# sergiventosa/ts-PWS

Measured on AMD Instinct MI355X. Metric: stacked samples/s (Morlet ts-PWS, 10k×131072) + % HBM roofline, 1/2/4/8 GPU, higher is better.
Workload: dtype f64; 1 GPU; 10000 traces/GPU x 131072 samples, Morlet w0=pi*sqrt(2/ln2) V=4 J=14, two-stage K=10 + unbiased phase coherence (BASELINE configs[2]); HBM-resident float32 traces; traces_total=10000, traces_per_gpu=10000, parallelism=one GPU: no collective, world_size=1

## Files before the change

### ts-pws_amd/csrc/inv_poly.h

```cpp
#pragma once

#define INV_R 8
#ifndef INV_UNIFORM
#define INV_UNIFORM 1
#endif

#ifndef FL_ABLATE
#define FL_ABLATE 0
#endif
#if FL_ABLATE
__device__ unsigned inv_class_mask = 0x7fu;
#endif

#define INV_QB 32
#define INV_WROWS (64 * INV_R + INV_QB + 16)
#define INV_WPAD(e) ((e) + ((e) >> 3))
#define INV_SLAB (INV_WROWS + INV_WROWS / 8 + 2)

struct OctDesc {
	unsigned s0, nv;
	unsigned D, Ns;
	unsigned DL, logDL, MC;
	unsigned ngw;
	unsigned wave_off;
	unsigned slot;
	unsigned gen, pad1;
};

#define INV_QSTEP(TP, YW)                                                                                     \
	if constexpr (QUAD) {                                                                                     \
		_Pragma("unroll") for (int c = 0; c < NREC; c++)                                                      \
			_Pragma("unroll") for (int r = 0; r < R; r++)                                                     \
				accq[c][r] = fma((TP).x, (YW).y, fma(-(TP).y, (YW).x, accq[c][r]));                             \
	}
template <int NREC, bool GEN, bool LDSW = false, bool QUAD = false>
__global__ void __launch_bounds__(256) k_inv_poly(const double2 *__restrict__ Y, size_t ncoef, unsigned N, const ScaleDesc *__restrict__ sc,
                                                  const OctDesc *__restrict__ oc, unsigned noct, const double2 *__restrict__ wd,
                                                  double *__restrict__ obuf, size_t slot_stride, unsigned total_waves, size_t y_coef,
                                                  size_t y_obuf, unsigned wave_base, size_t q_off = 0)
{
	Y += (size_t)blockIdx.y * y_coef; obuf += (size_t)blockIdx.y * y_obuf;
	constexpr int R = INV_R;
	const unsigned lane = threadIdx.x & 63;
	const unsigned wid = wave_base + blockIdx.x * 4 + __builtin_amdgcn_readfirstlane(threadIdx.x >> 6);
	if (wid >= total_waves) return;
	unsigned lo = 0, hi = noct;
	while (hi - lo > 1) {
		const unsigned mid = (lo + hi) >> 1;
		if (oc[mid].wave_off <= wid) lo = mid; else hi = mid;
	}
	const OctDesc o = oc[lo];
#if FL_ABLATE
	if (!((inv_class_mask >> o.logDL) & 1u)) return;
#endif
	const unsigned wl = wid - o.wave_off;
	const unsigned chunk = wl / o.ngw, gb = wl - chunk * o.ngw;
	const unsigned n0 = chunk * 64 + (lane & (o.DL - 1));
	const unsigned g = gb * (64u / o.DL) + (lane >> o.logDL);
	const bool live = n0 < o.D && g * R < o.Ns;
	const unsigned n0c = n0 < o.D ? n0 : 0;
	const unsigned D = o.D, Ns = o.Ns;

	double acc[NREC][R];
#pragma unroll
	for (int c = 0; c < NREC; c++)
#pragma unroll
		for (int r = 0; r < R; r++) acc[c][r] = 0;
	double accq[QUAD ? NREC : 1][R];
#pragma unroll
// ... 86 lines not shown
#pragma unroll
				for (int j = 0; j < R - 1; j++) {
					const bool in = idx >= 0 && idx < (long long)Ns;
#pragma unroll
					for (int c = 0; c < NREC; c++) yw[c][j] = in ? ys[(size_t)c * ncoef + (size_t)(in ? idx : 0)] : make_double2(0.0, 0.0);
					idx++;
				}
				unsigned l = mu;
				for (unsigned q = 0; q < d.Q + 1; q += R) {
#pragma unroll
					for (int u = 0; u < R; u++) {
						const bool in = idx >= 0 && idx < (long long)Ns;
#pragma unroll
						for (int c = 0; c < NREC; c++)
							yw[c][(u + R - 1) % R] = in ? ys[(size_t)c * ncoef + (size_t)(in ? idx : 0)] : make_double2(0.0, 0.0);
						idx++;
						double2 tp = ws[l < d.L ? l : d.L - 1];
						if (l < d.L) {
							tp.x *= gD; tp.y *= gD;
#pragma unroll
							for (int c = 0; c < NREC; c++)
#pragma unroll
								for (int r = 0; r < R; r++)
									acc[c][r] = fma(tp.x, yw[c][(u + r) % R].x, fma(tp.y, yw[c][(u + r) % R].y, acc[c][r]));
							INV_QSTEP(tp, yw[c][(u + r) % R])
						}
						l += D;
					}
				}
			}
		}
	} else if (INV_UNIFORM && o.DL == 64) {
	const unsigned gu = gb;
	for (unsigned v = 0; v < o.nv; v++) {
		const ScaleDesc d = sc[o.s0 + v];
		const double2 *ws = wd + d.tap_off;
		const double2 *ys = Y + d.coef_off;
		const long long t = (long long)n0c - d.cd;
		const long long a = t >= 0 ? t / D : -((-t + D - 1) / D);
		const unsigned rho = (unsigned)(t - a * (long long)D);
		const unsigned mu = rho ? D - rho : 0;
		const int idx = (int)a + (rho ? 1 : 0);
		const int A = __builtin_amdgcn_readfirstlane(idx);
		const unsigned shift = n0 < D ? (unsigned)(idx - A) : 0u;
		long long am = ((long long)A + (long long)gu * R) % (long long)Ns;
		if (am < 0) am += Ns;
		unsigned row = (unsigned)am;
		const double gD = d.gain * (double)D;
		double2 yw[NREC][R];
#pragma unroll
		for (int j = 0; j < R - 1; j++) {
#pragma unroll
			for (int c = 0; c < NREC; c++) yw[c][j] = ys[(size_t)c * ncoef + row];
			if (++row == Ns) row = 0;
		}
		unsigned l = mu - shift * D;
		for (unsigned q = 0; q < d.Q + 1; q += R) {
#pragma unroll
			for (int u = 0; u < R; u++) {
#pragma unroll
				for (int c = 0; c < NREC; c++) yw[c][(u + R - 1) % R] = ys[(size_t)c * ncoef + row];
				if (++row == Ns) row = 0;
				double2 tp = ws[l < d.L ? l : d.L - 1];
				if (l < d.L) {
					tp.x *= gD; tp.y *= gD;
#pragma unroll
					for (int c = 0; c < NREC; c++)
#pragma unroll
						for (int r = 0; r < R; r++)
							acc[c][r] = fma(tp.x, yw[c][(u + r) % R].x, fma(tp.y, yw[c][(u + r) % R].y, acc[c][r]));
					INV_QSTEP(tp, yw[c][(u + r) % R])
				}
				l += D;
			}
		}
	}
	} else {
	for (unsigned v = 0; v < o.nv; v++) {
		const ScaleDesc d = sc[o.s0 + v];
		const double2 *ws = wd + d.tap_off;
		const double2 *ys = Y + d.coef_off;
		const long long t = (long long)n0c - d.cd;
		long long a = t >= 0 ? t / D : -((-t + D - 1) / D);
		const unsigned rho = (unsigned)(t - a * (long long)D);
		const unsigned mu = rho ? D - rho : 0;
		a += (long long)g * R + (rho ? 1 : 0);
		long long am = a % (long long)Ns;
		if (am < 0) am += Ns;
		unsigned row = (unsigned)am;
		const double gD = d.gain * (double)D;
		double2 yw[NREC][R];
#pragma unroll
		for (int j = 0; j < R - 1; j++) {
#pragma unroll
			for (int c = 0; c < NREC; c++) yw[c][j] = ys[(size_t)c * ncoef + row];
			if (++row == Ns) row = 0;
		}
		unsigned l = mu, q = 0;
		for (; q + R <= d.Q; q += R) {
#pragma unroll
			for (int u = 0; u < R; u++) {
#pragma unroll
				for (int c = 0; c < NREC; c++) yw[c][(u + R - 1) % R] = ys[(size_t)c * ncoef + row];
				if (++row == Ns) row = 0;
				double2 tp = ws[l < d.L ? l : d.L - 1];
				if (l < d.L) {
					tp.x *= gD; tp.y *= gD;
#pragma unroll
// ... 149 lines not shown
```

### ts-pws_amd/csrc/forward.hip

```cpp
#include "tspws_internal.h"
#include <type_traits>

#ifndef FL_PASSES
#define FL_PASSES 2
#endif
#ifndef FL_WAVES
#define FL_WAVES 4
#endif
#ifndef FL_PASSES_FINE
#define FL_PASSES_FINE 1
#endif

template <typename TIn, bool BLOCK_PER_OUT>
__global__ void __launch_bounds__(256) k_fwd_generic(const TIn *__restrict__ x, size_t ld, unsigned N, const ScaleDesc *__restrict__ sc,
                                                     unsigned S, const double2 *__restrict__ w, double2 *__restrict__ Y, size_t ncoef,
                                                     unsigned long long first_coef, unsigned long long n_items)
{
	__shared__ double red[8];
	const unsigned lane = threadIdx.x & 63, wv = threadIdx.x >> 6;
	unsigned long long item = BLOCK_PER_OUT ? blockIdx.x : (unsigned long long)blockIdx.x * 4 + wv;
	if (item >= n_items) return;
	const unsigned long long ci = first_coef + item;
	const unsigned s = find_scale(sc, S, ci, false);
	const ScaleDesc d = sc[s];
// ... 22 lines not shown
			re = red[0] + red[2] + red[4] + red[6];
			im = red[1] + red[3] + red[5] + red[7];
			*out = make_double2(re, -im);
		}
	} else if (lane == 0) *out = make_double2(re, -im);
}

template <typename TIn>
static int forward_generic(tspws_hip_plan *p, const TIn *d_x, size_t ntr, size_t ld, double *d_Y, hipStream_t st)
{
	if (!p || !d_x || !d_Y) return fail(TSPWS_E_ARG, "forward: NULL");
	if (!ntr) return 0;
	HIP_TRY(hipSetDevice(p->device));
	unsigned s_long = p->S;
	for (unsigned s = 0; s < p->S; s++) if (p->sc[s].L > 2048) { s_long = s; break; }
	const unsigned long long n_short = s_long < p->S ? p->sc[s_long].coef_off : p->ncoef;
	const unsigned long long n_long = p->ncoef - n_short;
	for (size_t t0 = 0; t0 < ntr; t0 += 65535) {
		const unsigned ny = (unsigned)std::min<size_t>(ntr - t0, 65535);
		const TIn *xx = d_x + t0 * ld;
		double2 *yy = (double2 *)d_Y + t0 * p->ncoef;
		if (n_long)
			hipLaunchKernelGGL((k_fwd_generic<TIn, true>), dim3((unsigned)n_long, ny), dim3(256), 0, st, xx, ld, p->N, p->d_sc, p->S,
			                   p->d_w, yy, p->ncoef, n_short, n_long);
		if (n_short)
			hipLaunchKernelGGL((k_fwd_generic<TIn, false>), dim3((unsigned)((n_short + 3) / 4), ny), dim3(256), 0, st, xx, ld, p->N,
			                   p->d_sc, p->S, p->d_w, yy, p->ncoef, 0ull, n_short);
	}
	HIP_TRY(hipGetLastError());
	return 0;
}

#include "fwd_poly.h"
#include "fwd_lds.h"
#include "fwd_tl.h"
#include "fwd_gemm.h"
#include "spectral.h"

int tspws_engine_pin()
{
	static int eng = -2;
	if (eng == -2) {
		const char *e = getenv("TSPWS_ENGINE");
		eng = (!e || !*e || !strcmp(e, "auto")) ? 0 : !strcmp(e, "fir") ? 1 : !strcmp(e, "spectral") ? 2 : -1;
	}
	return eng;
}

static long tl_min_env()
{
	const char *e = sweep_env("TSPWS_TL_MIN");
	return e ? std::max(1, atoi(e)) : -1;
}

#ifndef FWD_LDS_MIN_NG
#define FWD_LDS_MIN_NG 8
#endif
#ifndef TL_MINNS0
#define TL_MINNS0 33
#endif
#ifndef FWD_STEPS_DEF
#define FWD_STEPS_DEF 32
#endif
#ifndef FWD_STEPS_TL
#define FWD_STEPS_TL 96
#endif
static int build_tl_forward(tspws_hip_plan *p, unsigned FWD_STEPS, unsigned MINNS, unsigned TLSTEPS, TlTable &T, unsigned spec_first = ~0u, unsigned spec_end = ~0u,
                            unsigned nblk_hint = 0);

int tspws_build_forward(tspws_hip_plan *p)
{
	const unsigned S = p->S;
	unsigned FWD_STEPS = FWD_STEPS_DEF;
	if (const char *e = sweep_env("TSPWS_FWD_STEPS")) FWD_STEPS = (unsigned)std::max(8, atoi(e));
	const unsigned R = 8, FL_SLOTS_HOST = FL_WAVES * FL_PASSES;
	unsigned woff = 0, boff = 0;
	unsigned long long poff = 0;
	for (unsigned s = 0; s < S; s++) {
		ScaleDesc &d = p->sc[s];
		d.Q = (d.L + d.D - 1) / d.D;
		unsigned dl = 1, lg = 0;
		while (dl < d.D && dl < 64) { dl <<= 1; lg++; }
		d.DL = dl; d.logDL = lg;
		d.MC = d.D > 64 ? (d.D + 63) / 64 : 1;
		const unsigned NG = (d.Ns + R - 1) / R, GW = 64 / d.DL;
		const bool pow2 = (d.D & (d.D - 1)) == 0;
		d.use_lds = (NG >= FWD_LDS_MIN_NG && (d.D >= 64 || pow2)) ? 1u : 0u;
		d.ngw = (NG + GW - 1) / GW;
		d.r16 = (!d.use_lds && d.DL == 64 && d.Ns >= 16) ? 1u : 0u;
		if (d.r16) d.ngw = (d.Ns + 15) / 16;
		unsigned cps;
		if (d.use_lds) cps = 1;
		else cps = std::max(1u, (FWD_STEPS + d.Q / 2) / std::max(1u, d.Q));
		d.cps = std::min(cps, d.MC);
		d.nsplit = (d.MC + d.cps - 1) / d.cps;
		d.wave_off = woff; d.lds_off = boff; d.part_off = poff;
		const unsigned slots = (d.D <= 4) ? FL_WAVES * FL_PASSES_FINE : FL_SLOTS_HOST;
		d.lds_bps = (NG + slots * GW - 1) / (slots * GW);
		if (d.use_lds) boff += d.lds_bps * d.nsplit; else woff += d.ngw * d.nsplit;
		poff += (unsigned long long)d.nsplit * d.Ns;
		d.fuse_ok = (d.use_lds && d.nsplit == 1) ? 1u : 0u;
		p->n_fusable += d.fuse_ok;
	}
	p->fwd_waves = woff; p->lds_blocks = boff; p->npart = poff;
	p->lds_qt = 24;
	for (unsigned s = 0; s < S; s++) if (p->sc[s].use_lds && p->sc[s].Q > 24 && p->sc[s].Q <= 32) p->lds_qt = 32;
	if (const char *e = sweep_env("TSPWS_FWD_QT")) { const int v = atoi(e); if (v == 24 || v == 32) p->lds_qt = (unsigned)v; }
	if (int rc = build_tl_forward(p, FWD_STEPS_TL, TL_MINNS0, 96, p->tl[0])) return rc;
	unsigned minns1 = 129, tlsteps1 = 48;
	if (const char *e = sweep_env("TSPWS_TLSTEPS")) tlsteps1 = (unsigned)std::max(8, atoi(e));
	if (const char *e = sweep_env("TSPWS_TL_MINNS1")) minns1 = (unsigned)std::max(9, atoi(e));
	return build_tl_forward(p, FWD_STEPS_TL, minns1, tlsteps1, p->tl[1]);
}

static int build_tl_forward(tspws_hip_plan *p, unsigned FWD_STEPS, unsigned MINNS, unsigned TLSTEPS, TlTable &T, unsigned spec_first, unsigned spec_end,
                            unsigned nblk_hint)
{
	T.minns = MINNS;
	T.sc = p->sc;
	std::vector<TLItem> items;
	std::vector<char> is_tl(p->S, 0);
	unsigned wg = 0;
	const unsigned S_fir = std::min(p->S, spec_first);
	for (unsigned s = 0; s < S_fir;) {
		unsigned e = s + 1;
		while (e < S_fir && p->sc[e].D == p->sc[s].D && p->sc[e].Ns == p->sc[s].Ns) e++;
		const unsigned D = p->sc[s].D, Ns = p->sc[s].Ns, nv = e - s;
		bool ok = Ns >= MINNS;
		std::vector<unsigned> a(nv), b(nv), qr(nv);
		for (unsigned v = 0; v < nv && ok; v++) {
			const ScaleDesc &d = p->sc[s + v];
			a[v] = (unsigned)d.c / D; b[v] = (unsigned)d.c % D;
			const long long num = (long long)d.L - 1 - (long long)b[v];
			const long long fl = num >= 0 ? num / (long long)D : -1;
			qr[v] = ((unsigned)(fl + 2) + 3) & ~3u;
			if (qr[v] > TL_QMAX) ok = false;
		}
// ... 72 lines not shown
	HIP_TRY(hipMalloc(&T.d_sc, p->S * sizeof(ScaleDesc)));
	HIP_TRY(hipMemcpy(T.d_sc, T.sc.data(), p->S * sizeof(ScaleDesc), hipMemcpyHostToDevice));
	if (T.gcoltiles) {
		std::vector<GemmCol> gc((size_t)T.gcoltiles * 16);
		memset(gc.data(), 0, gc.size() * sizeof(GemmCol));
		size_t i = 0;
		for (unsigned s = spec_end; s < p->S; s++) {
			const ScaleDesc &d = T.sc[s];
			for (unsigned k = 0; k < d.Ns; k++, i++) {
				GemmCol &g = gc[i];
				long long o = ((long long)d.c - (long long)k * (long long)d.D) % (long long)p->N;
				if (o < 0) o += p->N;
				g.L = d.L; g.o = (unsigned)o; g.Ns = d.Ns; g.tap_off = d.tap_off; g.dst = d.part_off + k;
			}
		}
		HIP_TRY(hipMalloc(&T.d_gcols, gc.size() * sizeof(GemmCol)));
		HIP_TRY(hipMemcpy(T.d_gcols, gc.data(), gc.size() * sizeof(GemmCol), hipMemcpyHostToDevice));
	}
	if (!T.n) return 0;
	HIP_TRY(hipMalloc(&T.d_items, items.size() * sizeof(TLItem)));
	HIP_TRY(hipMemcpy(T.d_items, items.data(), items.size() * sizeof(TLItem), hipMemcpyHostToDevice));
	HIP_TRY(hipFuncSetAttribute((const void *)k_fwd_tl<float>, hipFuncAttributeMaxDynamicSharedMemorySize, 160 * 1024));
	HIP_TRY(hipFuncSetAttribute((const void *)k_fwd_tl<double>, hipFuncAttributeMaxDynamicSharedMemorySize, 160 * 1024));
	return 0;
}

int tspws_build_tl_spectral(tspws_hip_plan *p, unsigned s_first, unsigned s_end, unsigned nblk_hint, TlTable &T)
{
	unsigned steps = 12;
	if (const char *e = sweep_env("TSPWS_SPEC_TLSTEPS")) steps = (unsigned)std::max(1, atoi(e));
	return build_tl_forward(p, FWD_STEPS_TL, TL_MINNS0, steps, T, s_first, s_end, nblk_hint);
}

struct LaunchRange { unsigned lds0, lds1, wav0, wav1, acc0, acc1; };
static LaunchRange launch_range(const tspws_hip_plan *p, ScaleRange rg)
{
	LaunchRange r;
	r.lds0 = rg.on() ? p->sc[rg.s0].lds_off : 0u;
	r.lds1 = rg.on() && rg.s1 < p->S ? p->sc[rg.s1].lds_off : p->lds_blocks;
	r.wav0 = rg.on() ? p->sc[rg.s0].wave_off : 0u;
	r.wav1 = rg.on() && rg.s1 < p->S ? p->sc[rg.s1].wave_off : p->fwd_waves;
	r.acc0 = rg.on() ? p->sc[rg.s0].acc2_off : 0u;
	r.acc1 = rg.on() && rg.s1 < p->S ? p->sc[rg.s1].acc2_off : p->acc2_blocks;
	return r;
}

template <typename TIn>
static void launch_poly2(const tspws_hip_plan *p, const TIn *d_x, size_t ld, size_t ntr, const ScaleDesc *d_sc, double2 *d_part, size_t npart, unsigned wav1,
                         unsigned wav0, hipStream_t st)
{
	for (size_t t0 = 0; t0 < ntr; t0 += 2 * 32768) {
		const unsigned nt = (unsigned)std::min<size_t>(ntr - t0, 2 * 32768);
		hipLaunchKernelGGL((k_fwd_poly<TIn, 2>), dim3((wav1 - wav0 + 3) / 4, (nt + 1) / 2), dim3(256), 0, st, d_x + t0 * ld, ld, nt, p->N, d_sc, p->S, p->d_w,
		                   d_part + t0 * npart, npart, wav1, wav0);
	}
}

template <typename TIn>
int tspws_forward_parts(tspws_hip_plan *p, const TIn *d_x, size_t ntr, size_t ld, double2 *d_part, hipStream_t st, FuseOut *fz, ScaleRange rg)
{
	if (fz) { fz->applied = false; fz->spec_first = p->S; }
	bool spec_join = false;
	hipStream_t fir = st;
	if constexpr (std::is_same<TIn, double>::value) {
		if (fz && fz->allow_spec && !rg.on() && fz->fin.OUT && fz->fin.nprev == 0 && ntr <= 512 && fz->tps) {
			static int min_rows = -1;
			static unsigned nsmax_env = 0;
			if (min_rows < 0) {
				const char *e = sweep_env("TSPWS_FEW_SPEC_MIN"); min_rows = e ? std::max(1, atoi(e)) : 64;
				if (const char *m = sweep_env("TSPWS_FEW_NSMAX")) nsmax_env = (unsigned)std::max(2, atoi(m));
			}
			if (ntr >= (size_t)min_rows && tspws_engine_pin() != 1 && !tspws_generic_forward()) {
				const unsigned sf = tspws_spectral_first_scale(p, nsmax_env ? nsmax_env : std::max(512u, (p->N + 15u) / 16u));
				if (sf < p->S && tspws_spectral_end_scale(p) == p->S) {
					SpecDecomp *dc = nullptr;
					int rc;
					if ((rc = tspws_spectral_decomp(p, sf, (unsigned)((ntr + 63) / 64), &dc, true))) return rc;
					static const bool serial = sweep_env("TSPWS_SPEC_PARALLEL") && !strcmp(sweep_env("TSPWS_SPEC_PARALLEL"), "0");
					hipEvent_t behind_tr = nullptr;
					if (!serial && sf > 0) {
						if ((rc = tspws_plan_stream(p, p->xs)) || (rc = tspws_plan_event(p->ev_xs2))) return rc;
						behind_tr = fz->ev_mid ? fz->ev_mid : p->ev_xs2;
					}
					if ((rc = tspws_spectral_rows_f64(p, dc, (const double *)d_x, ld, (unsigned)ntr, fz->tps, *fz, st, behind_tr))) return rc;
					fz->spec_first = sf;
					if (behind_tr) {
						if ((rc = tspws_fork(p, st, p->xs, p->ev_xs2, behind_tr))) return rc;
						fz->mid_recorded = behind_tr == fz->ev_mid;
						fir = p->xs;
					} else if (fz->ev_mid) { HIP_TRY(hipEventRecord(fz->ev_mid, st)); fz->mid_recorded = true; }
					if (sf == 0) { fz->applied = true; return 0; }
					rg.s0 = 0; rg.s1 = sf;
					spec_join = fir != st;
				}
			}
		}
	}
	const LaunchRange lr = launch_range(p, rg);
	const bool has_lds = lr.lds1 > lr.lds0, has_poly = lr.wav1 > lr.wav0;
	hipStream_t sp = fir;
#if FL_TIMING || FL_ABLATE
	static const bool serial = sweep_env("TSPWS_FWD_SERIAL") != nullptr;
#else
	constexpr bool serial = false;
#endif
	if (has_lds && has_poly && !serial) {
		if (int rc = tspws_fork(p, fir, p->side, p->ev_fork, fir == st ? p->le.ready : nullptr)) return rc;
		sp = p->side;
	}
	p->le.ready = nullptr;
	if (has_poly) {
		if (ntr == 1)
			hipLaunchKernelGGL((k_fwd_poly<TIn, 1>), dim3((lr.wav1 - lr.wav0 + 3) / 4, 1), dim3(256), 0, sp, d_x, ld, 1u, p->N, p->d_sc, p->S, p->d_w, d_part,
			                   p->npart, lr.wav1, lr.wav0);
		else launch_poly2<TIn>(p, d_x, ld, ntr, p->d_sc, d_part, p->npart, lr.wav1, lr.wav0, sp);
	}
	if (has_lds) {
		const bool fuse = fz && fz->accST && p->n_fusable;
		unsigned tps = (unsigned)std::min<size_t>(ntr, 32);
		while (tps > 1 && (size_t)p->lds_blocks * ((ntr + tps - 1) / tps) < 2048) tps = (tps + 1) / 2;
		if (fuse) tps = fz->tps;
		const size_t per_launch = (size_t)tps * 65535;
		for (size_t t0 = 0; t0 < ntr; t0 += per_launch) {
			const unsigned nt = (unsigned)std::min<size_t>(ntr - t0, per_launch);
			const dim3 grid(lr.lds1 - lr.lds0, (nt + tps - 1) / tps);
			double2 *aS = fuse ? fz->accST + (t0 / tps) * fz->stride : nullptr, *aP = fuse ? fz->accPS + (t0 / tps) * fz->stride : nullptr;
			const size_t astr = fuse ? fz->stride : 0;
			FuseFinal ff;
			if (fuse && fz->fin.OUT && t0 == 0 && ntr <= per_launch) ff = fz->fin;
#define FL_LAUNCH(F, QT) hipLaunchKernelGGL((k_fwd_lds<TIn, F, QT>), grid, dim3(FL_NT), FL_LDS_BYTES_(QT), fir, d_x + t0 * ld, ld, nt, tps, p->N, p->d_sc, p->S, \
			                            p->d_w, d_part + t0 * p->npart, p->npart, aS, aP, astr, lr.lds0, ff)
			if (p->lds_qt == 32) { if (fuse) FL_LAUNCH(true, 32); else FL_LAUNCH(false, 32); }
			else { if (fuse) FL_LAUNCH(true, 24); else FL_LAUNCH(false, 24); }
#undef FL_LAUNCH
		}
		if (fuse) fz->applied = true;
	}
	if (sp != fir) if (int rc = tspws_join(sp, fir, p->ev_join)) return rc;
	if (spec_join) {
		if (fz && fz->defer_fir_join) fz->fir_stream = p->xs;
		else if (int rc = tspws_join(p->xs, st, p->ev_xs1)) return rc;
	}
	HIP_TRY(hipGetLastError());
	return 0;
// ... 369 lines not shown
```

### ts-pws_amd/csrc/plan.hip

```cpp
#include "tspws_internal.h"

static thread_local std::string g_err;

extern "C" const char *tspws_hip_last_error(void) { return g_err.c_str(); }

int tspws_fail(int code, const char *what, hipError_t e)
{
	g_err = what;
	if (e != hipSuccess) { g_err += ": "; g_err += hipGetErrorString(e); }
	return code;
}

int tspws_scratch(tspws_hip_plan *p, int slot, size_t bytes, void **out)
{
	if (p->scr_bytes[slot] < bytes) {
		void *fresh = nullptr;
		HIP_TRY(hipMalloc(&fresh, bytes));
		if (p->scr[slot]) {
			if (slot == SCR_P || slot == SCR_STPS || slot == SCR_JKP) p->retired.push_back(p->scr[slot]);
			else (void)hipFree(p->scr[slot]);
		}
		if (slot == SCR_TAB) p->ck_dev = false;
		if (slot == SCR_TAB || slot == SCR_JKTAB) p->jk_gen = 0;
		p->scr[slot] = fresh;
// ... 121 lines not shown
		}
	}
	w[t] = make_double2(re, im);
	wd[d.tap_off + (d.L - 1 - l)] = make_double2(re, -im);
}

static double cpsi_host(int type, double w0)
{
	if (type == -3) return (4. / 3.) * sqrt(TSPWS_PI);
	double acc = 0;
	for (double om = 0.01; om < 100; om += 0.01) {
		double d = om - w0;
		d *= d;
		acc += exp(-d) / om;
	}
	return acc * (0.01 * sqrt(TSPWS_PI) / 2);
}

extern "C" int tspws_hip_device_count(void)
{
	int n = 0;
	if (hipGetDeviceCount(&n) != hipSuccess) return 0;
	return n;
}

extern "C" int tspws_hip_plan_create(tspws_hip_plan **out, int type, unsigned J, unsigned V, unsigned N, double s0,
                                     double b0, double w0, int uni, int device)
{
	if (!out) return fail(TSPWS_E_ARG, "plan_create: NULL plan pointer");
	*out = nullptr;
	if (type > -1 || type < -3) return fail(TSPWS_E_FRAME, "plan_create: only complex families -1/-2/-3");
	if (V == 0 || J == 0 || N == 0) return fail(TSPWS_E_FRAME, "plan_create: empty frame (J, V and N must be > 0)");
	if (tspws_engine_pin() < 0) return fail(TSPWS_E_ARG, "plan_create: TSPWS_ENGINE must be fir, spectral or auto");
	if (tspws_hip_device_count() <= device) return fail(TSPWS_E_NODEV, "plan_create: no such HIP device");
	HIP_TRY(hipSetDevice(device));

	tspws_hip_plan *p = new (std::nothrow) tspws_hip_plan;
	if (!p) return fail(TSPWS_E_NOMEM, "plan_create: host allocation");
	p->device = device; p->type = type; p->V = V; p->J = J; p->N = N; p->S = J * V;
	p->s0 = s0; p->b0 = uni ? 1.0 : b0; p->w0 = w0;
	p->Cpsi = cpsi_host(type, w0);
	const unsigned S = p->S;
	p->sc.resize(S);
	double scv = s0;
	const double ratio = pow(2.0, 1.0 / (double)V);
	for (unsigned s = 0; s < S; s++) { p->sc[s].scale = scv; scv *= ratio; }
	double step = s0 * p->b0;
	for (unsigned j = 0, s = 0; j < J; j++) {
		const unsigned d = uni ? 1u : (step < 1.0 ? 1u : (unsigned)step);
		for (unsigned v = 0; v < V; v++) p->sc[s++].D = d;
		step *= 2.0;
	}
	unsigned long long toff = 0, coff = 0;
	for (unsigned s = 0; s < S; s++) {
		ScaleDesc &d = p->sc[s];
		const unsigned len = 2u * (unsigned)ceil(5.0 * d.scale) + 1u;
		d.L = len > N ? N : len;
		d.c = (int)(d.L / 2u);
		d.cd = (int)d.L - 1 - d.c;
		d.Ns = (N + d.D - 1u) / d.D;
		d.tap_off = toff; d.coef_off = coff;
		d.gain = log(2.0) / (2 * p->Cpsi * V * d.scale);
		toff += d.L; coff += d.Ns;
	}
	p->ntaps = toff; p->ncoef = coff;
	if (int rc = tspws_build_forward(p)) { tspws_hip_plan_destroy(p); return rc; }
// ... 9 lines not shown
	if ((e = hipMalloc(&p->d_sc, S * sizeof(ScaleDesc))) != hipSuccess ||
	    (e = hipMalloc(&p->d_w, p->ntaps * sizeof(double2))) != hipSuccess ||
	    (e = hipMalloc(&p->d_wd, p->ntaps * sizeof(double2))) != hipSuccess ||
	    (e = hipMemcpy(p->d_sc, p->sc.data(), S * sizeof(ScaleDesc), hipMemcpyHostToDevice)) != hipSuccess) {
		tspws_hip_plan_destroy(p);
		return fail(e == hipErrorOutOfMemory ? TSPWS_E_NOMEM : TSPWS_E_HIP, "plan_create: device tables", e);
	}
	if (int rc = tspws_build_inverse(p)) { tspws_hip_plan_destroy(p); return rc; }
	const unsigned nb = (unsigned)((p->ntaps + 255) / 256);
	hipLaunchKernelGGL(k_gen_taps, dim3(nb), dim3(256), 0, 0, p->d_sc, S, type, w0, (unsigned long long)p->ntaps, p->d_w, p->d_wd);
	if ((e = hipGetLastError()) != hipSuccess || (e = hipDeviceSynchronize()) != hipSuccess) {
		tspws_hip_plan_destroy(p);
		return fail(e == hipErrorNoBinaryForGpu ? TSPWS_E_NODEV : TSPWS_E_HIP, "plan_create: tap kernel", e);
	}
	*out = p;
	return 0;
}

extern "C" void tspws_hip_plan_destroy(tspws_hip_plan *p)
{
	if (!p) return;
	(void)hipSetDevice(p->device);
	for (int i = 0; i < SCR_N; i++) if (p->scr[i]) (void)hipFree(p->scr[i]);
	for (void *b : p->retired) (void)hipFree(b);
	for (hipEvent_t e : p->prof_ev) (void)hipEventDestroy(e);
	for (hipEvent_t e : p->stage_ev) (void)hipEventDestroy(e);
	for (hipEvent_t e : {p->ck_ev, p->ev_fork, p->ev_join, p->ev_xs0, p->ev_xs1, p->ev_xs2, p->ev_mid, p->ev_lin}) if (e) (void)hipEventDestroy(e);
	for (hipStream_t st : {p->side, p->xs, p->xf}) if (st) (void)hipStreamDestroy(st);
	if (p->d_oc) (void)hipFree(p->d_oc);
	tspws_bands_destroy(p);
	tspws_spectral_destroy(p);
	for (TlTable &T : p->tl) { if (T.d_sc) (void)hipFree(T.d_sc); if (T.d_items) (void)hipFree(T.d_items); }
	if (p->d_sc) (void)hipFree(p->d_sc);
	if (p->d_w) (void)hipFree(p->d_w);
	if (p->d_wd) (void)hipFree(p->d_wd);
	delete p;
}

extern "C" int tspws_hip_plan_info(const tspws_hip_plan *p, tspws_hip_frame_info *i)
{
	if (!p || !i) return fail(TSPWS_E_ARG, "plan_info: NULL");
	i->type = p->type; i->S = p->S; i->V = p->V; i->J = p->J; i->N = p->N;
	i->s0 = p->s0; i->b0 = p->b0; i->w0 = p->w0; i->Cpsi = p->Cpsi;
	i->ncoef = p->ncoef; i->ntaps = p->ntaps; i->device = p->device;
	return 0;
}

extern "C" int tspws_hip_plan_tables(const tspws_hip_plan *p, double *scale, unsigned *L, int *c, int *cd, unsigned *D, unsigned *Ns)
{
	if (!p) return fail(TSPWS_E_ARG, "plan_tables: NULL");
	for (unsigned s = 0; s < p->S; s++) {
		if (scale) scale[s] = p->sc[s].scale;
		if (L) L[s] = p->sc[s].L;
		if (c) c[s] = p->sc[s].c;
		if (cd) cd[s] = p->sc[s].cd;
		if (D) D[s] = p->sc[s].D;
		if (Ns) Ns[s] = p->sc[s].Ns;
	}
	return 0;
}

extern "C" int tspws_hip_plan_taps(const tspws_hip_plan *p, double *h_w, double *h_wd)
{
	if (!p) return fail(TSPWS_E_ARG, "plan_taps: NULL");
	HIP_TRY(hipSetDevice(p->device));
	if (h_w) HIP_TRY(hipMemcpy(h_w, p->d_w, p->ntaps * sizeof(double2), hipMemcpyDeviceToHost));
// ... 94 lines not shown
```

### ts-pws_amd/csrc/tspws_internal.h

```cpp
#pragma once

#include <hip/hip_runtime.h>

#include <algorithm>
#include <cmath>
#include <cstdio>
#include <cstdlib>
#include <cstring>
#include <string>
#include <vector>

#include "tspws_hip.h"
#include "column_runs.h"

#ifndef TSPWS_PI
#define TSPWS_PI 3.14159265358979328
#endif

int tspws_fail(int code, const char *what, hipError_t e = hipSuccess);
#define fail tspws_fail

#define HIP_TRY(expr)                                                              \
	do {                                                                           \
		hipError_t e_ = (expr);                                                    \
		if (e_ != hipSuccess) return tspws_fail(e_ == hipErrorOutOfMemory ? TSPWS_E_NOMEM : TSPWS_E_HIP, #expr, e_); \
	} while (0)

static inline hipStream_t S_(void *s) { return (hipStream_t)s; }

#ifdef TSPWS_SWEEPS
static inline const char *sweep_env(const char *name) { return getenv(name); }
#else
static inline const char *sweep_env(const char *) { return nullptr; }
#endif

struct ScaleDesc {
	unsigned L, D, Ns;
	int c, cd;
	unsigned Q;
	unsigned long long tap_off, coef_off;
	double scale, gain;
	unsigned DL, logDL;
	unsigned MC, cps, nsplit;
	unsigned ngw;
	unsigned wave_off;
// ... 63 lines not shown

struct OctDesc;
struct TLItem;

struct GemmCol;
struct TlTable {
	unsigned minns = 0;
	std::vector<ScaleDesc> sc;
	ScaleDesc *d_sc = nullptr;
	TLItem *d_items = nullptr;
	unsigned n = 0, wgs = 0, waves = 0, acc2_blocks = 0;
	size_t npart = 0, lds = 0;
	GemmCol *d_gcols = nullptr;
	unsigned gcoltiles = 0, gKS = 0, gKC = 0;
};

struct SpecDecomp;

struct TlPass {
	SpecDecomp *dc = nullptr;
	const TlTable *T = nullptr;
	size_t batch = 0;
	void *xT = nullptr;
	double2 *planes = nullptr, *part = nullptr, *gsum = nullptr;
};

struct tspws_hip_plan {
	int device = 0, type = -1;
	unsigned S = 0, V = 0, J = 0, N = 0;
	double s0 = 0, b0 = 0, w0 = 0, Cpsi = 0;
	size_t ncoef = 0, ntaps = 0;
	size_t npart = 0;
	unsigned fwd_waves = 0;
	unsigned acc_blocks = 0;
	unsigned acc2_blocks = 0;
	unsigned lds_blocks = 0;
	unsigned lds_qt = 24;
	unsigned n_fusable = 0;
	TlTable tl[2];
	std::vector<SpecDecomp *> spec;
	std::vector<unsigned> oc_s0, oc_nv, oc_wave_off, oc_nwaves, oc_gen;
	std::vector<unsigned> og_s0, og_nv;
	unsigned inv_waves_lds = 0;
	unsigned inv_waves = 0, inv_waves_fast = 0, inv_noct = 0, inv_ngeneric = 0;
	OctDesc *d_oc = nullptr;
	struct BandTables *bands = nullptr;
	std::vector<ScaleDesc> sc;
	ScaleDesc *d_sc = nullptr;
	double2 *d_w = nullptr, *d_wd = nullptr;
	void *scr[SCR_N] = {nullptr};
	size_t scr_bytes[SCR_N] = {0};
	hipStream_t side = nullptr;
	hipEvent_t ev_fork = nullptr, ev_join = nullptr;
	hipStream_t xs = nullptr;
	hipEvent_t ev_xs0 = nullptr, ev_xs1 = nullptr, ev_xs2 = nullptr;
	hipEvent_t ev_mid = nullptr;
	hipEvent_t ev_lin = nullptr;
	struct LaunchEvents { hipEvent_t first_start = nullptr, last_stop = nullptr, ready = nullptr, call_end = nullptr; } le;
	std::vector<hipEvent_t> prof_ev;
	size_t prof_used = 0;
	std::vector<Chunk> chunks;
	std::vector<unsigned> row_first;
	size_t ck_mtr = 0, ck_first = 0, ck_glob = 0;
	unsigned ck_K = 0;
	bool ck_valid = false, ck_dev = false;
	hipEvent_t ck_ev = nullptr;
// ... 93 lines not shown
		return make_double2(st.x * a / M, st.y * a / M);
	}
	const double iK = 1. / K, iK1 = 1. / (Kb - 1), iM = 1. / M;
	const double px = ps.x * iK, py = ps.y * iK;
	a = px * px + py * py;
	a = (Kb * a - 1) * iK1;
	return make_double2(st.x * a * iM, st.y * a * iM);
}

__device__ __forceinline__ double2 weight_value(const double2 st, const double2 ps, const int mode, const double K, const double M, const double wu)
{
	return weight_value_eff(st, ps, mode, K, K, M, wu);
}
#endif

int  tspws_build_forward(tspws_hip_plan *p);
template <typename TIn>
int  tspws_forward_parts(tspws_hip_plan *p, const TIn *d_x, size_t ntr, size_t ld, double2 *d_part, hipStream_t st, FuseOut *fz, ScaleRange rg);
template <typename TIn>
int  tspws_tl_pass_setup(tspws_hip_plan *p, size_t ntr, size_t nslots, TlPass &P);
template <typename TIn>
int  tspws_tl_pass_transform(tspws_hip_plan *p, const TlPass &P, const TIn *xb, size_t ld, unsigned nb, hipStream_t st);
template <typename TIn>
int  tspws_stacks(tspws_hip_plan *p, const TIn *d_x, size_t ntr, size_t ld, double *d_ST, double *d_PS, hipStream_t st, bool keep,
                  const WeightArgs *wa, bool *weighted, ScaleRange rg);
unsigned tspws_first_unfused_scale(const tspws_hip_plan *p);
void tspws_launch_accumulate(tspws_hip_plan *p, const double2 *part, unsigned nb, double2 *ST, double2 *PS, int zero_first, const FuseOut *fz,
                             unsigned nslices, hipStream_t st, unsigned nbatch, size_t y_part, size_t y_stack, const TlTable *tl, const WeightArgs *wa,
                             ScaleRange rg, const AccExtra *ex = nullptr);
bool tspws_fused_forward(const tspws_hip_plan *p);
bool tspws_many_trace_path(const tspws_hip_plan *p, size_t ntr);
unsigned tspws_spectral_choice(const tspws_hip_plan *p, size_t ntr);
size_t tspws_part_budget_bytes();
int  tspws_engine_pin();
bool tspws_generic_forward();
unsigned tspws_spectral_first_scale(const tspws_hip_plan *p, unsigned nsmax);
int  tspws_spectral_decomp(tspws_hip_plan *p, unsigned s_first, unsigned nblk_hint, SpecDecomp **out, bool few = false);
int  tspws_spectral_rows_f64(tspws_hip_plan *p, SpecDecomp *dc, const double *d_x, size_t ld, unsigned ntr, unsigned tps, const FuseOut &fz, hipStream_t st,
                             hipEvent_t after_transposition = nullptr);
int  tspws_build_tl_spectral(tspws_hip_plan *p, unsigned s_first, unsigned s_end, unsigned nblk_hint, TlTable &T);
void tspws_spectral_geometry(const tspws_hip_plan *p, unsigned *NT, unsigned *s_end, unsigned *cneg);
unsigned tspws_spectral_end_scale(const tspws_hip_plan *p);
struct SpecRowsOut;
template <typename TIn>
int  tspws_spectral_run(tspws_hip_plan *p, SpecDecomp *dc, const TIn *xT, unsigned TP, unsigned ntr, double2 *ST, double2 *PS, size_t stride, double2 *Y, hipStream_t st,
                        const SpecRowsOut *ro = nullptr, unsigned tps = 0, unsigned ncol = 0);
template <typename TIn>
int  tspws_spectral_transpose(tspws_hip_plan *p, const TIn *d_x, size_t ld, unsigned ntr, TIn *xT, unsigned TP, hipStream_t st);
void tspws_spectral_destroy(tspws_hip_plan *p);
int  tspws_build_inverse(tspws_hip_plan *p);
size_t tspws_inverse_row_bytes(const tspws_hip_plan *p);
int  tspws_weight_mode(double wu, int unbiased, unsigned K);
void tspws_weight_batched(tspws_hip_plan *p, double2 *OUT, const double2 *ST, const double2 *PS, int mode, double K, double wu, const double *d_Mv,
                          unsigned nb, size_t y_out, size_t y_stack, hipStream_t st, double M = 0.0);
int  tspws_inverse_pair_out(tspws_hip_plan *p, const double2 *Y, float *d_ts, float *d_ls, float mtr, hipStream_t st);
int  tspws_inverse_scales(tspws_hip_plan *p, const double2 *Y, double *x2, hipStream_t st, ScaleRange rg);
int  tspws_inverse_pairs_early(tspws_hip_plan *p, const double2 *Y, unsigned nb, unsigned s_split, hipStream_t early, bool *done);
int  tspws_inverse_pairs_late(tspws_hip_plan *p, const double2 *Y, double *x, unsigned nb, unsigned s_split, hipStream_t st);
bool tspws_generic_inverse();
struct BandOut {
	double *re = nullptr, *im = nullptr;
	float *ts = nullptr, *ls = nullptr, *ts_env = nullptr, *ls_env = nullptr;
	const unsigned *d_row = nullptr, *d_cnt = nullptr;
	unsigned row0 = 0, cnt0 = 1;
};
int  tspws_bands_check(const tspws_hip_plan *p, const tspws_band *bands, unsigned R, const char *who);
// ... 26 lines not shown
```

Baseline: 1349 billion samples/s.

## Software-pipeline uniform DL=64 inverse path with cooperative row loads and readlane broadcast

For the non-QUAD uniform DL=64 branch, the inner loop is restructured so each lane loads one double of the coefficient window and the values are broadcast to all lanes with readlane. The taps and rows for the next group are prefetched one iteration ahead, and the prefetch crosses scale boundaries. This is meant to hide global-load latency and to remove redundant per-lane loads of the same coefficient rows. Launch bounds are also raised to a minimum of 4 blocks per CU for the simple variants, which caps register use and may cause spills. The lane-to-element mapping assumes the window fits in 64 lanes (R*NREC*2 <= 64).

```diff
diff --git a/ts-pws_amd/csrc/inv_poly.h b/ts-pws_amd/csrc/inv_poly.h
--- a/ts-pws_amd/csrc/inv_poly.h
+++ b/ts-pws_amd/csrc/inv_poly.h
@@ -34,7 +34,7 @@
 				accq[c][r] = fma((TP).x, (YW).y, fma(-(TP).y, (YW).x, accq[c][r]));                             \
 	}
 template <int NREC, bool GEN, bool LDSW = false, bool QUAD = false>
-__global__ void __launch_bounds__(256) k_inv_poly(const double2 *__restrict__ Y, size_t ncoef, unsigned N, const ScaleDesc *__restrict__ sc,
+__global__ void __launch_bounds__(256, (GEN || LDSW || QUAD) ? 1 : 4) k_inv_poly(const double2 *__restrict__ Y, size_t ncoef, unsigned N, const ScaleDesc *__restrict__ sc,
                                                   const OctDesc *__restrict__ oc, unsigned noct, const double2 *__restrict__ wd,
                                                   double *__restrict__ obuf, size_t slot_stride, unsigned total_waves, size_t y_coef,
                                                   size_t y_obuf, unsigned wave_base, size_t q_off = 0)
@@ -187,6 +187,7 @@
 		}
 	} else if (INV_UNIFORM && o.DL == 64) {
 	const unsigned gu = gb;
+	if constexpr (QUAD) {
 	for (unsigned v = 0; v < o.nv; v++) {
 		const ScaleDesc d = sc[o.s0 + v];
 		const double2 *ws = wd + d.tap_off;
@@ -229,6 +230,87 @@
 				l += D;
 			}
 		}
+	}
+	} else {
+	constexpr int PER = 2 * NREC;
+	const unsigned ec = (lane / 2) % NREC, ex = lane & 1;
+	const unsigned ejm = (lane / PER) % Ns, adv7 = (unsigned)(R - 1) % Ns, adv8 = (unsigned)R % Ns;
+	const double2 *fws = wd;
+	const double *fys = (const double *)Y;
+	unsigned fv = 0, fq = 0, fQ = 0, fl = 0, fL = 1, frow = 0, nl = 0;
+	double ngD = 0, pre = 0;
+	auto rows = [&](unsigned adv) -> double {
+		unsigned rw = frow + ejm;
+		rw = rw >= Ns ? rw - Ns : rw;
+		const double x = fys[2 * ((size_t)ec * ncoef + rw) + ex];
+		frow += adv;
+		frow = frow >= Ns ? frow - Ns : frow;
+		return x;
+	};
+	auto enter = [&](unsigned v) {
+		const ScaleDesc d = sc[o.s0 + v];
+		const long long t = (long long)n0c - d.cd;
+		const long long a = t >= 0 ? t / D : -((-t + D - 1) / D);
+		const unsigned rho = (unsigned)(t - a * (long long)D);
+		const unsigned mu = rho ? D - rho : 0;
+		const int idx = (int)a + (rho ? 1 : 0);
+		const int A = __builtin_amdgcn_readfirstlane(idx);
+		const unsigned shift = n0 < D ? (unsigned)(idx - A) : 0u;
+		long long am = ((long long)A + (long long)gu * R) % (long long)Ns;
+		if (am < 0) am += Ns;
+		frow = (unsigned)am;
+		ngD = d.gain * (double)D;
+		nl = mu - shift * D;
+		fws = wd + d.tap_off; fys = (const double *)(Y + d.coef_off); fl = nl; fL = d.L; fQ = d.Q; fq = 0;
+		pre = rows(adv7);
+	};
+	double2 tn[R];
+	double rn;
+	auto request = [&]() {
+#pragma unroll
+		for (int u = 0; u < R; u++) {
+			const unsigned lu = fl + (unsigned)u * D;
+			tn[u] = fws[lu < fL ? lu : fL - 1];
+		}
+		rn = rows(adv8);
+		fl += (unsigned)R * D; fq += R;
+	};
+	if (o.nv) { enter(0); request(); }
+	for (unsigned v = 0; v < o.nv; v++) {
+		const double gD = ngD;
+		const unsigned L = fL, Q = fQ;
+		unsigned l = nl;
+		double2 yw[NREC][R];
+#pragma unroll
+		for (int j = 0; j < R - 1; j++)
+#pragma unroll
+			for (int c = 0; c < NREC; c++)
+				yw[c][j] = make_double2(readlane_f64(pre, (j * NREC + c) * 2), readlane_f64(pre, (j * NREC + c) * 2 + 1));
+		for (unsigned q = 0; q < Q + 1; q += R) {
+			double2 tp[R];
+#pragma unroll
+			for (int u = 0; u < R; u++) tp[u] = tn[u];
+			const double rp = rn;
+			if (fq >= fQ + 1 && fv + 1 < o.nv) enter(++fv);
+			request();
+			__builtin_amdgcn_sched_barrier(0);
+#pragma unroll
+			for (int u = 0; u < R; u++) {
+#pragma unroll
+				for (int c = 0; c < NREC; c++)
+					yw[c][(u + R - 1) % R] = make_double2(readlane_f64(rp, (u * NREC + c) * 2), readlane_f64(rp, (u * NREC + c) * 2 + 1));
+				if (l < L) {
+					const double2 tg = make_double2(tp[u].x * gD, tp[u].y * gD);
+#pragma unroll
+					for (int c = 0; c < NREC; c++)
+#pragma unroll
+						for (int r = 0; r < R; r++)
+							acc[c][r] = fma(tg.x, yw[c][(u + r) % R].x, fma(tg.y, yw[c][(u + r) % R].y, acc[c][r]));
+				}
+				l += D;
+			}
+		}
+	}
 	}
 	} else {
 	for (unsigned v = 0; v < o.nv; v++) {
```

Result: no change. 1347 billion samples/s, median of 2 (-0.1%).

## Add register-blocked coarse forward kernel for long-decimation scales

Applied to the files above, without the earlier changes.

Adds a new forward kernel for non-LDS scales with D>=64 and few outputs. Each wave keeps a sliding window of decimated input samples in registers and accumulates up to 32 outputs for one or two traces, reusing every tap load across all outputs and traces. When NS*D is a multiple of N it uses a ring mode that loads the inputs once. These scales are removed from the poly wave table, and an env pin can restore the direct path. The cost is heavy register pressure from the large accumulator arrays, which may hurt occupancy.

```diff
diff --git a/ts-pws_amd/csrc/coarse_plan.h b/ts-pws_amd/csrc/coarse_plan.h
--- /dev/null
+++ b/ts-pws_amd/csrc/coarse_plan.h
@@ -0,0 +1,94 @@
+#pragma once
+#include <algorithm>
+#include <cstring>
+#include <vector>
+
+struct FwdSplit {
+	unsigned Q, DL, logDL, MC;
+	unsigned use_lds, ngw, r16;
+	unsigned cps, nsplit;
+};
+
+inline FwdSplit fwd_split(unsigned L, unsigned D, unsigned Ns, unsigned steps, unsigned min_ng)
+{
+	const unsigned R = 8;
+	FwdSplit f;
+	f.Q = (L + D - 1) / D;
+	unsigned dl = 1, lg = 0;
+	while (dl < D && dl < 64) { dl <<= 1; lg++; }
+	f.DL = dl; f.logDL = lg;
+	f.MC = D > 64 ? (D + 63) / 64 : 1;
+	const unsigned NG = (Ns + R - 1) / R, GW = 64 / f.DL;
+	const bool pow2 = (D & (D - 1)) == 0;
+	f.use_lds = (NG >= min_ng && (D >= 64 || pow2)) ? 1u : 0u;
+	f.ngw = (NG + GW - 1) / GW;
+	f.r16 = (!f.use_lds && f.DL == 64 && Ns >= 16) ? 1u : 0u;
+	if (f.r16) f.ngw = (Ns + 15) / 16;
+	unsigned cps;
+	if (f.use_lds) cps = 1;
+	else cps = std::max(1u, (steps + f.Q / 2) / std::max(1u, f.Q));
+	f.cps = std::min(cps, f.MC);
+	f.nsplit = (f.MC + f.cps - 1) / f.cps;
+	return f;
+}
+
+struct CoarseItem {
+	unsigned s;
+	unsigned NS, B;
+	unsigned ring;
+	unsigned wave_off;
+	unsigned nwaves;
+};
+
+enum { COARSE_DIRECT = 0, COARSE_WHOLE = 1, COARSE_AUTO = 2, COARSE_BAD = -1 };
+
+inline int coarse_pin_parse(const char *e)
+{
+	if (!e || !*e || !strcmp(e, "auto")) return COARSE_AUTO;
+	if (!strcmp(e, "direct")) return COARSE_DIRECT;
+	if (!strcmp(e, "whole")) return COARSE_WHOLE;
+	return COARSE_BAD;
+}
+
+inline unsigned coarse_ns(unsigned Ns) { return Ns <= 8 ? 8u : Ns <= 16 ? 16u : 32u; }
+
+inline bool coarse_qualifies(unsigned N, unsigned L, unsigned D, unsigned Ns, const FwdSplit &f)
+{
+	if (f.use_lds || D < 64 || Ns > 32) return false;
+	if ((unsigned long long)N * 8ull >= 0x80000000ull) return false;
+	return ((unsigned long long)L + (unsigned long long)(f.Q + 2u * coarse_ns(Ns)) * D + 64ull) * 16ull < 0x80000000ull;
+}
+
+struct CoarsePlan {
+	std::vector<CoarseItem> items;
+	std::vector<unsigned char> on;
+	unsigned waves = 0;
+	std::vector<unsigned> poly_off;
+	void range(unsigned s0, unsigned s1, unsigned &w0, unsigned &w1) const
+	{
+		w0 = w1 = waves;
+		for (size_t i = items.size(); i-- > 0;) {
+			if (items[i].s >= s1) w1 = items[i].wave_off;
+			if (items[i].s >= s0) w0 = items[i].wave_off;
+		}
+	}
+};
+
+inline CoarsePlan coarse_plan_build(unsigned N, unsigned S, const unsigned *L, const unsigned *D, const unsigned *Ns, const FwdSplit *split, bool enabled)
+{
+	CoarsePlan P;
+	P.on.assign(S, 0);
+	for (unsigned s = 0; s < S && enabled; s++) {
+		if (!coarse_qualifies(N, L[s], D[s], Ns[s], split[s])) continue;
+		CoarseItem it;
+		it.s = s; it.NS = coarse_ns(Ns[s]); it.B = it.NS == 32 ? 1u : 2u;
+		it.ring = ((unsigned long long)it.NS * D[s]) % N == 0 ? 1u : 0u;
+		it.wave_off = P.waves; it.nwaves = split[s].nsplit * (2u / it.B);
+		P.waves += it.nwaves;
+		P.items.push_back(it);
+		P.on[s] = 1;
+	}
+	P.poly_off.assign(S + 1, 0);
+	for (unsigned s = 0; s < S; s++) P.poly_off[s + 1] = P.poly_off[s] + ((split[s].use_lds || P.on[s]) ? 0u : split[s].ngw * split[s].nsplit);
+	return P;
+}
diff --git a/ts-pws_amd/csrc/forward.hip b/ts-pws_amd/csrc/forward.hip
--- a/ts-pws_amd/csrc/forward.hip
+++ b/ts-pws_amd/csrc/forward.hip
@@ -78,6 +78,7 @@
 }
 
 #include "fwd_poly.h"
+#include "fwd_coarse.h"
 #include "fwd_lds.h"
 #include "fwd_tl.h"
 #include "fwd_gemm.h"
@@ -93,6 +94,13 @@
 	return eng;
 }
 
+int tspws_coarse_pin()
+{
+	static int pin = -2;
+	if (pin == -2) pin = coarse_pin_parse(getenv("TSPWS_FWD_COARSE"));
+	return pin;
+}
+
 static long tl_min_env()
 {
 	const char *e = sweep_env("TSPWS_TL_MIN");
@@ -120,35 +128,35 @@
 	unsigned FWD_STEPS = FWD_STEPS_DEF;
 	if (const char *e = sweep_env("TSPWS_FWD_STEPS")) FWD_STEPS = (unsigned)std::max(8, atoi(e));
 	const unsigned R = 8, FL_SLOTS_HOST = FL_WAVES * FL_PASSES;
-	unsigned woff = 0, boff = 0;
+	unsigned boff = 0;
 	unsigned long long poff = 0;
+	std::vector<FwdSplit> split(S);
+	std::vector<unsigned> vL(S), vD(S), vNs(S);
+	for (unsigned s = 0; s < S; s++) {
+		const ScaleDesc &d = p->sc[s];
+		vL[s] = d.L; vD[s] = d.D; vNs[s] = d.Ns;
+		split[s] = fwd_split(d.L, d.D, d.Ns, FWD_STEPS, FWD_LDS_MIN_NG);
+	}
+	p->coarse = coarse_plan_build(p->N, S, vL.data(), vD.data(), vNs.data(), split.data(), tspws_coarse_pin() != COARSE_DIRECT);
 	for (unsigned s = 0; s < S; s++) {
 		ScaleDesc &d = p->sc[s];
-		d.Q = (d.L + d.D - 1) / d.D;
-		unsigned dl = 1, lg = 0;
-		while (dl < d.D && dl < 64) { dl <<= 1; lg++; }
-		d.DL = dl; d.logDL = lg;
-		d.MC = d.D > 64 ? (d.D + 63) / 64 : 1;
+		const FwdSplit &f = split[s];
+		d.Q = f.Q; d.DL = f.DL; d.logDL = f.logDL; d.MC = f.MC;
+		d.use_lds = f.use_lds; d.ngw = f.ngw; d.r16 = f.r16; d.cps = f.cps; d.nsplit = f.nsplit;
 		const unsigned NG = (d.Ns + R - 1) / R, GW = 64 / d.DL;
-		const bool pow2 = (d.D & (d.D - 1)) == 0;
-		d.use_lds = (NG >= FWD_LDS_MIN_NG && (d.D >= 64 || pow2)) ? 1u : 0u;
-		d.ngw = (NG + GW - 1) / GW;
-		d.r16 = (!d.use_lds && d.DL == 64 && d.Ns >= 16) ? 1u : 0u;
-		if (d.r16) d.ngw = (d.Ns + 15) / 16;
-		unsigned cps;
-		if (d.use_lds) cps = 1;
-		else cps = std::max(1u, (FWD_STEPS + d.Q / 2) / std::max(1u, d.Q));
-		d.cps = std::min(cps, d.MC);
-		d.nsplit = (d.MC + d.cps - 1) / d.cps;
-		d.wave_off = woff; d.lds_off = boff; d.part_off = poff;
+		d.wave_off = p->coarse.poly_off[s]; d.lds_off = boff; d.part_off = poff;
 		const unsigned slots = (d.D <= 4) ? FL_WAVES * FL_PASSES_FINE : FL_SLOTS_HOST;
 		d.lds_bps = (NG + slots * GW - 1) / (slots * GW);
-		if (d.use_lds) boff += d.lds_bps * d.nsplit; else woff += d.ngw * d.nsplit;
+		if (d.use_lds) boff += d.lds_bps * d.nsplit;
 		poff += (unsigned long long)d.nsplit * d.Ns;
 		d.fuse_ok = (d.use_lds && d.nsplit == 1) ? 1u : 0u;
 		p->n_fusable += d.fuse_ok;
 	}
-	p->fwd_waves = woff; p->lds_blocks = boff; p->npart = poff;
+	p->fwd_waves = p->coarse.poly_off[S]; p->lds_blocks = boff; p->npart = poff;
+	if (!p->coarse.items.empty()) {
+		HIP_TRY(hipMalloc(&p->d_coarse, p->coarse.items.size() * sizeof(CoarseItem)));
+		HIP_TRY(hipMemcpy(p->d_coarse, p->coarse.items.data(), p->coarse.items.size() * sizeof(CoarseItem), hipMemcpyHostToDevice));
+	}
 	p->lds_qt = 24;
 	for (unsigned s = 0; s < S; s++) if (p->sc[s].use_lds && p->sc[s].Q > 24 && p->sc[s].Q <= 32) p->lds_qt = 32;
 	if (const char *e = sweep_env("TSPWS_FWD_QT")) { const int v = atoi(e); if (v == 24 || v == 32) p->lds_qt = (unsigned)v; }
@@ -287,10 +295,11 @@
 	return build_tl_forward(p, FWD_STEPS_TL, TL_MINNS0, steps, T, s_first, s_end, nblk_hint);
 }
 
-struct LaunchRange { unsigned lds0, lds1, wav0, wav1, acc0, acc1; };
+struct LaunchRange { unsigned lds0, lds1, wav0, wav1, acc0, acc1, cw0, cw1; };
 static LaunchRange launch_range(const tspws_hip_plan *p, ScaleRange rg)
 {
 	LaunchRange r;
+	p->coarse.range(rg.on() ? rg.s0 : 0u, rg.on() ? rg.s1 : p->S, r.cw0, r.cw1);
 	r.lds0 = rg.on() ? p->sc[rg.s0].lds_off : 0u;
 	r.lds1 = rg.on() && rg.s1 < p->S ? p->sc[rg.s1].lds_off : p->lds_blocks;
 	r.wav0 = rg.on() ? p->sc[rg.s0].wave_off : 0u;
@@ -352,19 +361,27 @@
 		}
 	}
 	const LaunchRange lr = launch_range(p, rg);
-	const bool has_lds = lr.lds1 > lr.lds0, has_poly = lr.wav1 > lr.wav0;
+	const bool has_lds = lr.lds1 > lr.lds0, has_coarse = lr.cw1 > lr.cw0, has_poly = lr.wav1 > lr.wav0 || has_coarse;
 	hipStream_t sp = fir;
 #if FL_TIMING || FL_ABLATE
 	static const bool serial = sweep_env("TSPWS_FWD_SERIAL") != nullptr;
 #else
 	constexpr bool serial = false;
 #endif
-	if (has_lds && has_poly && !serial) {
+	static const bool coarse_serial = sweep_env("TSPWS_FWD_COARSE_SERIAL") && !strcmp(sweep_env("TSPWS_FWD_COARSE_SERIAL"), "1");
+	if (has_lds && has_poly && !serial && !coarse_serial) {
 		if (int rc = tspws_fork(p, fir, p->side, p->ev_fork, fir == st ? p->le.ready : nullptr)) return rc;
 		sp = p->side;
 	}
 	p->le.ready = nullptr;
-	if (has_poly) {
+	if (has_coarse) {
+		for (size_t t0 = 0; t0 < ntr; t0 += 2 * 32768) {
+			const unsigned nt = (unsigned)std::min<size_t>(ntr - t0, 2 * 32768);
+			hipLaunchKernelGGL((k_fwd_coarse<TIn>), dim3((lr.cw1 - lr.cw0 + 3) / 4, (nt + 1) / 2), dim3(256), 0, sp, d_x + t0 * ld, ld, nt, p->N, p->d_sc,
+			                   (const CoarseItem *)p->d_coarse, (unsigned)p->coarse.items.size(), p->d_w, d_part + t0 * p->npart, p->npart, lr.cw1, lr.cw0);
+		}
+	}
+	if (lr.wav1 > lr.wav0) {
 		if (ntr == 1)
 			hipLaunchKernelGGL((k_fwd_poly<TIn, 1>), dim3((lr.wav1 - lr.wav0 + 3) / 4, 1), dim3(256), 0, sp, d_x, ld, 1u, p->N, p->d_sc, p->S, p->d_w, d_part,
 			                   p->npart, lr.wav1, lr.wav0);
diff --git a/ts-pws_amd/csrc/fwd_coarse.h b/ts-pws_amd/csrc/fwd_coarse.h
--- /dev/null
+++ b/ts-pws_amd/csrc/fwd_coarse.h
@@ -0,0 +1,145 @@
+#pragma once
+#include "coarse_plan.h"
+
+#define FWD_COARSE_BS 4
+
+template <typename TIn, int NS, int B, bool RING>
+__device__ __forceinline__ void fwd_coarse_wave(const TIn *__restrict__ x, size_t ld, unsigned ntr, unsigned N, const ScaleDesc &d,
+                                                const double2 *__restrict__ w, double2 *__restrict__ part, size_t npart, const unsigned split,
+                                                const unsigned t0, const unsigned lane)
+{
+	constexpr int BS = FWD_COARSE_BS;
+	static_assert(NS % BS == 0 && NS % 8 == 0, "the ring is walked in blocks of BS steps and reduced eight outputs at a time");
+	const double2 *ws = w + d.tap_off;
+	const unsigned Nb = N * (unsigned)sizeof(TIn), Dwb = (d.D % N) * (unsigned)sizeof(TIn), D16 = d.D * 16u;
+	__amdgpu_buffer_rsrc_t rx[B], rw;
+#pragma unroll
+	for (int b = 0; b < B; b++) {
+		unsigned t = t0 + (unsigned)b;
+		if (t >= ntr) t = ntr - 1;
+		rx[b] = __builtin_amdgcn_make_buffer_rsrc((void *)(x + (size_t)t * ld), 0, Nb, 0x00020000);
+	}
+	rw = __builtin_amdgcn_make_buffer_rsrc((void *)ws, 0, d.L * 16u, 0x00020000);
+	auto ldx = [&](const int b, const unsigned off) -> double {
+		if constexpr (sizeof(TIn) == 8) return (double)__builtin_bit_cast(TIn, __builtin_amdgcn_raw_buffer_load_b64(rx[b], off, 0, 0));
+		else return (double)__builtin_bit_cast(TIn, __builtin_amdgcn_raw_buffer_load_b32(rx[b], off, 0, 0));
+	};
+	auto ldw = [&](const unsigned off) -> double2 {
+		const auto raw = __builtin_amdgcn_raw_buffer_load_b128(rw, off, 0, 0);
+		return make_double2(__hiloint2double((int)raw[1], (int)raw[0]), __hiloint2double((int)raw[3], (int)raw[2]));
+	};
+
+	double ar[B][NS], ai[B][NS];
+#pragma unroll
+	for (int b = 0; b < B; b++)
+#pragma unroll
+		for (int r = 0; r < NS; r++) { ar[b][r] = 0; ai[b][r] = 0; }
+
+	for (unsigned ci = 0; ci < d.cps; ci++) {
+		const unsigned chunk = split * d.cps + ci;
+		if (chunk >= d.MC) break;
+		const unsigned m = chunk * 64 + lane;
+		const bool mvalid = m < d.D;
+		const unsigned mm = mvalid ? m : 0;
+		unsigned row = wrap_index((long long)mm - d.c, N) * (unsigned)sizeof(TIn);
+		unsigned tb = mvalid ? mm * 16u : 0x80000000u;
+		double xw[B][NS];
+#pragma unroll
+		for (int j = 0; j < (RING ? NS : NS - 1); j++) {
+#pragma unroll
+			for (int b = 0; b < B; b++) xw[b][j] = ldx(b, row);
+			row += Dwb; row = min(row, row - Nb);
+		}
+		double2 tpn[BS];
+		if constexpr (RING) {
+#pragma unroll
+			for (int u = 0; u < BS; u++) { tpn[u] = ldw(tb); tb += D16; }
+		}
+		for (unsigned q = 0; q < d.Q; q += NS) {
+#pragma unroll
+			for (int h = 0; h < NS / BS; h++) {
+				if (q + (unsigned)(h * BS) < d.Q) {
+					const unsigned nsteps = d.Q - q - (unsigned)(h * BS);
+					double2 tp[BS];
+					double xn[B][BS];
+					if constexpr (RING) {
+#pragma unroll
+						for (int u = 0; u < BS; u++) tp[u] = tpn[u];
+						if (nsteps > (unsigned)BS) {
+#pragma unroll
+							for (int u = 0; u < BS; u++) { tpn[u] = ldw(tb); tb += D16; }
+						}
+					} else {
+#pragma unroll
+						for (int u = 0; u < BS; u++) {
+#pragma unroll
+							for (int b = 0; b < B; b++) xn[b][u] = ldx(b, row);
+							row += Dwb; row = min(row, row - Nb);
+							tp[u] = ldw(tb); tb += D16;
+						}
+					}
+#pragma unroll
+					for (int u = 0; u < BS; u++) {
+						if ((unsigned)u < nsteps) {
+							const int sidx = h * BS + u;
+							if constexpr (!RING) {
+#pragma unroll
+								for (int b = 0; b < B; b++) xw[b][(sidx + NS - 1) % NS] = xn[b][u];
+							}
+#pragma unroll
+							for (int b = 0; b < B; b++)
+#pragma unroll
+								for (int r = 0; r < NS; r++) {
+									ar[b][r] = fma(xw[b][(sidx + r) % NS], tp[u].x, ar[b][r]);
+									ai[b][r] = fma(xw[b][(sidx + r) % NS], tp[u].y, ai[b][r]);
+								}
+						}
+					}
+				}
+			}
+		}
+	}
+
+	const unsigned o = ((lane >> 5) & 1) * 8 + ((lane >> 4) & 1) * 4 + ((lane >> 3) & 1) * 2 + ((lane >> 2) & 1);
+#pragma unroll
+	for (int b = 0; b < B; b++) {
+#pragma unroll
+		for (int half = 0; half < NS / 8; half++) {
+			double v16[16];
+#pragma unroll
+			for (int r = 0; r < 8; r++) { v16[2 * r] = ar[b][half * 8 + r]; v16[2 * r + 1] = ai[b][half * 8 + r]; }
+			const double sum = valu_reduce16(v16, lane);
+			const unsigned t = t0 + (unsigned)b, k = (unsigned)(half * 8) + (o >> 1);
+			if ((lane & 3) == 0 && t < ntr && k < d.Ns) {
+				double *dst = (double *)(part + (size_t)t * npart + d.part_off + (size_t)split * d.Ns);
+				dst[(size_t)k * 2 + (o & 1)] = (o & 1) ? -sum : sum;
+			}
+		}
+	}
+}
+
+template <typename TIn>
+__global__ void __launch_bounds__(256) k_fwd_coarse(const TIn *__restrict__ x, size_t ld, unsigned ntr, unsigned N, const ScaleDesc *__restrict__ sc,
+                                                    const CoarseItem *__restrict__ items, unsigned nitems, const double2 *__restrict__ w,
+                                                    double2 *__restrict__ part, size_t npart, unsigned wav1, unsigned wav0)
+{
+	const unsigned lane = threadIdx.x & 63;
+	const unsigned wid = wav0 + blockIdx.x * 4 + __builtin_amdgcn_readfirstlane(threadIdx.x >> 6);
+	if (wid >= wav1) return;
+	unsigned lo = 0, hi = nitems;
+	while (hi - lo > 1) {
+		const unsigned mid = (lo + hi) >> 1;
+		if (items[mid].wave_off <= wid) lo = mid; else hi = mid;
+	}
+	const CoarseItem it = items[lo];
+	const ScaleDesc d = sc[it.s];
+	const unsigned wl = wid - it.wave_off, split = wl % d.nsplit, tsel = wl / d.nsplit;
+	const unsigned t0 = blockIdx.y * 2 + tsel;
+	if (t0 >= ntr) return;
+#define FC_RUN(NS_, B_) do { if (it.ring) fwd_coarse_wave<TIn, NS_, B_, true>(x, ld, ntr, N, d, w, part, npart, split, t0, lane); \
+                             else fwd_coarse_wave<TIn, NS_, B_, false>(x, ld, ntr, N, d, w, part, npart, split, t0, lane); } while (0)
+	if (it.NS == 8) FC_RUN(8, 2);
+	else if (it.NS == 16) FC_RUN(16, 2);
+	else FC_RUN(32, 1);
+#undef FC_RUN
+}
diff --git a/ts-pws_amd/csrc/plan.hip b/ts-pws_amd/csrc/plan.hip
--- a/ts-pws_amd/csrc/plan.hip
+++ b/ts-pws_amd/csrc/plan.hip
@@ -177,6 +177,7 @@
 	if (type > -1 || type < -3) return fail(TSPWS_E_FRAME, "plan_create: only complex families -1/-2/-3");
 	if (V == 0 || J == 0 || N == 0) return fail(TSPWS_E_FRAME, "plan_create: empty frame (J, V and N must be > 0)");
 	if (tspws_engine_pin() < 0) return fail(TSPWS_E_ARG, "plan_create: TSPWS_ENGINE must be fir, spectral or auto");
+	if (tspws_coarse_pin() == COARSE_BAD) return fail(TSPWS_E_ARG, "plan_create: TSPWS_FWD_COARSE must be direct, whole or auto");
 	if (tspws_hip_device_count() <= device) return fail(TSPWS_E_NODEV, "plan_create: no such HIP device");
 	HIP_TRY(hipSetDevice(device));
 
@@ -252,6 +253,7 @@
 	tspws_spectral_destroy(p);
 	for (TlTable &T : p->tl) { if (T.d_sc) (void)hipFree(T.d_sc); if (T.d_items) (void)hipFree(T.d_items); }
 	if (p->d_sc) (void)hipFree(p->d_sc);
+	if (p->d_coarse) (void)hipFree(p->d_coarse);
 	if (p->d_w) (void)hipFree(p->d_w);
 	if (p->d_wd) (void)hipFree(p->d_wd);
 	delete p;
diff --git a/ts-pws_amd/csrc/tspws_internal.h b/ts-pws_amd/csrc/tspws_internal.h
--- a/ts-pws_amd/csrc/tspws_internal.h
+++ b/ts-pws_amd/csrc/tspws_internal.h
@@ -11,6 +11,7 @@
 #include <vector>
 
 #include "tspws_hip.h"
+#include "coarse_plan.h"
 #include "column_runs.h"
 
 #ifndef TSPWS_PI
@@ -140,6 +141,8 @@
 	size_t ncoef = 0, ntaps = 0;
 	size_t npart = 0;
 	unsigned fwd_waves = 0;
+	CoarsePlan coarse;
+	CoarseItem *d_coarse = nullptr;
 	unsigned acc_blocks = 0;
 	unsigned acc2_blocks = 0;
 	unsigned lds_blocks = 0;
@@ -299,6 +302,7 @@
 bool tspws_many_trace_path(const tspws_hip_plan *p, size_t ntr);
 unsigned tspws_spectral_choice(const tspws_hip_plan *p, size_t ntr);
 size_t tspws_part_budget_bytes();
+int  tspws_coarse_pin();
 int  tspws_engine_pin();
 bool tspws_generic_forward();
 unsigned tspws_spectral_first_scale(const tspws_hip_plan *p, unsigned nsmax);
```

Result: no change. 1352 billion samples/s before, 1359 billion samples/s after (median of 6 runs) (+0.5%).
